# balazs-bamer/cdpr-simulation

Measured on AMD Instinct MI355X. Metric: CDPR sim-steps/sec (whole node), 65 536 parallel 8-cable robots, 1 ms dt, higher is better.
Workload: dtype f32

## Files before the change

cdpr-simulation_amd/csrc/cdpr_onestep_kernel.hpp:

```cpp
#pragma once
#include "cdpr_step_kernel.hpp"

namespace cdpr {

CDPR_DEV void row_to_lds(const float4* src, float4* dst_row) {
  __builtin_amdgcn_global_load_lds((const __attribute__((address_space(1))) void*)src, (__attribute__((address_space(3))) void*)dst_row, 16, 0, 0);
}


template <int NP, bool PR = false, bool FULL = false>
CDPR_DEV void pid_pairs(const StepArgs& a, int calls, bool is_vel, const v2f (&desired)[NP], const v2f (&actual)[NP], const v2f (&win)[NP][kWin],
                        v2f (&ierr)[NP], v2f (&f)[NP], v2f (&e_new)[NP], float& dbg_p, float& dbg_i, float& dbg_d, bool is_force = false) {
  const PidCoef c = pid_coef<PR>(a, is_vel);
  const bool run = (!PR || calls != 0) && !is_force;
  const bool full = FULL || calls >= c.nbuf;
  const float (&wt)[kWin + 2] = a.wrow;
  v2f error[NP], acc[NP];
#pragma unroll
  for (int k = 0; k < NP; ++k) {
    error[k] = desired[k] - actual[k];
    acc[k] = splat(wt[kWin]) * error[k];
  }
#pragma unroll
  for (int j = 0; j < kWin; ++j) {
// ... 328 lines not shown
      ik_pairs<N, false>(lds + again, s.px, s.py, s.pz, s.qx, s.qy, s.qz, s.qw, len2, jac, l02);
    }
    float w[6];
    jt_times<NP>(jac, tens, w);
    w[0] = a.fgx - w[0];
    w[1] = a.fgy - w[1];
    w[2] = a.fgz - w[2];
    w[3] = -w[3];
    w[4] = -w[4];
    w[5] = -w[5];
    integrate(a, s, w);
  }
  if (PERSIST && more) {
    constexpr int kDmaOps = kCtrl + kCmdRows;
    static_assert(kDmaOps < 64, "vmcnt is a 6-bit counter");
    if (run_pid)
      __builtin_amdgcn_s_waitcnt(vmcnt_imm(kDmaOps));
    else
      __builtin_amdgcn_s_waitcnt(vmcnt_imm(0));
    asm volatile("" : "+a"(n0), "+a"(n1), "+a"(n2), "+a"(n3), "+a"(n4));
  }
  if (live) {
    CDPR_STORE_STATE(a.state, st, 0, woff, make_float4(s.px, s.py, s.pz, s.qx));
    CDPR_STORE_STATE(a.state, st, 1, woff, make_float4(s.qy, s.qz, s.qw, s.vx));
    CDPR_STORE_STATE(a.state, st, 2, woff, make_float4(s.vy, s.vz, s.wx, s.wy));
    CDPR_STORE_STATE(a.state, st, 3, woff, make_float4(s.wz, fkx, fky, fkz));
    if (FK) CDPR_STORE_STATE(a.state, st, 4, woff, make_float4(fkqx, fkqy, fkqz, fkqw));
  }
  CDPR_STAMP(7);
  if (!(PERSIST && more)) break;
  blk = nblk;
  r = nr;
  rr = nrr;
  live = r < a.batch;
  off = rr * 16u, woff = r * 16u;
  p0 = make_float4(n0.x, n0.y, n0.z, n0.w), p1 = make_float4(n1.x, n1.y, n1.z, n1.w), p2 = make_float4(n2.x, n2.y, n2.z, n2.w);
  p3 = make_float4(n3.x, n3.y, n3.z, n3.w), p4 = make_float4(n4.x, n4.y, n4.z, n4.w);
  staged = run_pid;
  }
}

#ifndef CDPR_CTL_LOAD_DELAY
#define CDPR_CTL_LOAD_DELAY 8
#endif
#ifndef CDPR_SPLIT_PRIO
#define CDPR_SPLIT_PRIO 1
#endif
#ifndef CDPR_STEADY_SHARED_IK
#define CDPR_STEADY_SHARED_IK 1
#endif
#ifndef CDPR_STEADY_NEWTON_WRITTEN_OUT
#define CDPR_STEADY_NEWTON_WRITTEN_OUT 1
#endif
constexpr int kIkRows = 7;
#ifdef CDPR_STAMPS
#define CDPR_SPLIT_STAMP(i)                                                                                          \
  do {                                                                                                               \
    __builtin_amdgcn_sched_barrier(0);                                                                               \
    if (a.stamps && lane == 0) a.stamps[(size_t)blockIdx.x * 8 + (i)] = __builtin_amdgcn_s_memrealtime();           \
    __builtin_amdgcn_sched_barrier(0);                                                                               \
  } while (0)
#else
#define CDPR_SPLIT_STAMP(i) do { } while (0)
#endif
#if defined(CDPR_STAMPS) && defined(CDPR_STAMPS_ITER)
#define CDPR_CTL_STAMP(i) do { } while (0)
#else
#define CDPR_CTL_STAMP(i) CDPR_SPLIT_STAMP(i)
#endif

template <int N, int XS, int ES, bool RAISED = true, bool STEADY = false>
CDPR_DEV void split_estimator_wave(const StepArgs& a, float* geo, float gval, uint32_t lane, bool live, size_t st, uint32_t off, uint32_t woff,
                                   const float4& p0, const float4& p1, const float4& p3, const v2f* x_force, v2f* x_tension, float* x_est,
                                   v2f* x_ik = nullptr) {
  constexpr int NP = cable_pairs(N);
#if defined(CDPR_STAMPS) && defined(CDPR_STAMPS_CLOCK)
  const unsigned long long clk0 = __builtin_amdgcn_s_memtime();
#endif
#if CDPR_SPLIT_PRIO == 1 || CDPR_SPLIT_PRIO == 4
  if (RAISED) __builtin_amdgcn_s_setprio(3);
#elif CDPR_SPLIT_PRIO == 3 || CDPR_SPLIT_PRIO == 5
  if (RAISED) __builtin_amdgcn_s_setprio(2);
#endif
  const float4 p4 = load_slot(a.state, st, 4, off);
  if (lane < NP * kGeomFloatsPerPair) geo[lane] = gval;
  __builtin_amdgcn_fence(__ATOMIC_RELEASE, "wavefront");
  __builtin_amdgcn_wave_barrier();
  __builtin_amdgcn_fence(__ATOMIC_ACQUIRE, "wavefront");
  float fkx = p3.y, fky = p3.z, fkz = p3.w, fkqx = p4.x, fkqy = p4.y, fkqz = p4.z, fkqw = p4.w;
  v2f len[NP];
  {
    v2f jac[NP][6], l0[NP];
    ik_pairs<N, false>(geo, p0.x, p0.y, p0.z, p0.w, p1.x, p1.y, p1.z, len, jac, l0);
    if (STEADY && CDPR_STEADY_SHARED_IK) {
#pragma unroll
      for (int k = 0; k < NP; ++k) {
        x_ik[(kIkRows * k) * 64 + lane] = len[k];
#pragma unroll
        for (int c = 0; c < 6; ++c) x_ik[(kIkRows * k + 1 + c) * 64 + lane] = jac[k][c];
      }
      __builtin_amdgcn_fence(__ATOMIC_RELEASE, "workgroup");
      __builtin_amdgcn_s_waitcnt(0xC07F);
      __builtin_amdgcn_s_barrier();
    }
  }
  float fk_res = 0.f;
  int fk_it = 0;
  v2f jest[NP][6];
  {
    v2f elen[NP], unused[NP];
    if (STEADY && CDPR_STEADY_NEWTON_WRITTEN_OUT) {
#pragma unroll
      for (int it = 0; it < 4; ++it) {
        ik_pairs<N, false>(geo, fkx, fky, fkz, fkqx, fkqy, fkqz, fkqw, elen, jest, unused);
        v2f res[NP];
#pragma unroll
        for (int k = 0; k < NP; ++k) res[k] = len[k] - elen[k];
        float g[6];
        jt_times<NP>(jest, res, g);
        normal_solve<NP>(jest, a.fk_lambda, g);
        fkx += g[0];
        fky += g[1];
        fkz += g[2];
        quat_apply_rotvec(fkqx, fkqy, fkqz, fkqw, g[3], g[4], g[5]);
#ifdef CDPR_STAMPS_ITER
        if (it < 3) {
          asm volatile("" ::"v"(fkqw));
          __builtin_amdgcn_sched_barrier(0);
          if (a.stamps && lane == 0) a.stamps[(size_t)blockIdx.x * 8 + 4 + it] = __builtin_amdgcn_s_memrealtime();
          __builtin_amdgcn_sched_barrier(0);
        }
#endif
      }
      fk_it = 4;
    } else {
      bool active = true;
      for (int it = 0; it < a.fk_iters; ++it) {
        ik_pairs<N, false>(geo, fkx, fky, fkz, fkqx, fkqy, fkqz, fkqw, elen, jest, unused);
        v2f res[NP];
        v2f rm = splat(0.f);
#pragma unroll
        for (int k = 0; k < NP; ++k) {
          res[k] = len[k] - elen[k];
          rm = max2(rm, abs2(res[k]));
        }
        active = active && !(fmaxf(rm.x, rm.y) < a.fk_tol);
        float g[6];
        jt_times<NP>(jest, res, g);
        normal_solve<NP>(jest, a.fk_lambda, g);
        if (active) {
          fkx += g[0];
          fky += g[1];
          fkz += g[2];
          quat_apply_rotvec(fkqx, fkqy, fkqz, fkqw, g[3], g[4], g[5]);
          ++fk_it;
        }
#ifdef CDPR_STAMPS_ITER
        if (it < 3) {
          asm volatile("" ::"v"(fkqw));
          __builtin_amdgcn_sched_barrier(0);
          if (a.stamps && lane == 0) a.stamps[(size_t)blockIdx.x * 8 + 4 + it] = __builtin_amdgcn_s_memrealtime();
          __builtin_amdgcn_sched_barrier(0);
        }
#endif
      }
    }
    ik_pairs<N, false>(geo, fkx, fky, fkz, fkqx, fkqy, fkqz, fkqw, elen, jest, unused);
    v2f rm = splat(0.f);
#pragma unroll
    for (int k = 0; k < NP; ++k) rm = max2(rm, abs2(len[k] - elen[k]));
    fk_res = fmaxf(rm.x, rm.y);
  }
  if (live) store_slot_aux<CDPR_SPLIT_PLAT_AUX>(a.state, st, 4, woff, make_float4(fkqx, fkqy, fkqz, fkqw));
  CDPR_SPLIT_STAMP(1);
  v2f td_l[6][3];
  float td_invd[6];
  normal_matrix_pk<NP, false>(jest, 0.f, td_l);
  chol_factor_pk(td_l, td_invd);
  __builtin_amdgcn_s_waitcnt(0xC07F);
  __builtin_amdgcn_s_barrier();
  CDPR_SPLIT_STAMP(2);
  __builtin_amdgcn_fence(__ATOMIC_ACQUIRE, "workgroup");
  v2f f[NP], df[NP], t_out[NP];
#pragma unroll
  for (int k = 0; k < NP; ++k) {
    f[k] = x_force[k * XS + lane];
    df[k] = f[k] - splat(a.td_mid);
  }
  int td_flag = 0;
  {
    float g[6];
    jt_times<NP>(jest, df, g);
    chol_apply_pk(td_l, td_invd, g);
#pragma unroll
    for (int k = 0; k < NP; ++k) {
      v2f t = splat(a.td_mid);
#pragma unroll
      for (int c = 0; c < 6; ++c) t = fma2(g[c], jest[k][c], t);
      const v2f tc = max2(min2(t, splat(a.td_max)), splat(a.td_min));
      td_flag |= (tc.x != t.x) ? 1 : 0;
      if (2 * k + 1 < N) td_flag |= (tc.y != t.y) ? 1 : 0;
      t_out[k] = tc;
    }
  }
#pragma unroll
  for (int k = 0; k < NP; ++k) x_tension[k * XS + lane] = t_out[k];
  x_est[0 * ES + lane] = fkx;
  x_est[1 * ES + lane] = fky;
  x_est[2 * ES + lane] = fkz;
  x_est[3 * ES + lane] = fk_res;
  x_est[4 * ES + lane] = (float)fk_it;
  x_est[5 * ES + lane] = (float)td_flag;
  __builtin_amdgcn_fence(__ATOMIC_RELEASE, "workgroup");
  __builtin_amdgcn_s_waitcnt(0xC07F);
  CDPR_SPLIT_STAMP(3);
#if defined(CDPR_STAMPS) && defined(CDPR_STAMPS_CLOCK)
  if (a.stamps && lane == 0) a.stamps[(size_t)blockIdx.x * 8 + 7] = __builtin_amdgcn_s_memtime() - clk0;
#endif
  __builtin_amdgcn_s_barrier();
}

template <int N, bool PR, bool STEADY, bool VEL>
CDPR_DEV void split_controller_wave(const StepArgs& a, float* geo, float gval, uint32_t lane, uint32_t r, uint32_t rr, bool live, size_t st, uint32_t off,
                                    uint32_t woff, const float4& p0, const float4& p1, const float4& p2, const float4& p3, v2f* x_force, const v2f* x_tension,
                                    const float* x_est, const v2f* x_ik = nullptr) {
  static_assert(!(STEADY && PR), "the steady instantiation serves uniform handles");
  constexpr int NP = cable_pairs(N);
  constexpr int P = plat_slots(true);
  constexpr int G = joint_groups(N);
  constexpr int NH = (NP + 1) / 2;
#if CDPR_SPLIT_PRIO == 2 || CDPR_SPLIT_PRIO == 5
  __builtin_amdgcn_s_setprio(3);
#endif
#if CDPR_CTL_LOAD_DELAY > 0
  __builtin_amdgcn_s_sleep(CDPR_CTL_LOAD_DELAY);
#endif
  float4 wraw[NP][5], hraw[NH];
#pragma unroll
  for (int k = 0; k < NP; ++k) {
#pragma unroll
    for (int m = 0; m < 5; ++m) wraw[k][m] = load_slot(a.state, st, P + 5 * k + m, off);
  }
#pragma unroll
  for (int g = 0; g < NH; ++g) hraw[g] = load_slot(a.state, st, P + 5 * NP + g, off);
  v2f desired[NP];
#pragma unroll
  for (int k = 0; k < NP; ++k) desired[k] = splat(0.f);
  const float* cp = a.cmd + (size_t)rr * N;
  if (N % 4 == 0) {
#pragma unroll
    for (int g = 0; g < N / 4; ++g) {
      const float4 v = reinterpret_cast<const float4*>(cp)[g];
      desired[2 * g] = (v2f){v.x, v.y};
      desired[2 * g + 1] = (v2f){v.z, v.w};
    }
  } else {
#pragma unroll
    for (int i = 0; i < N; ++i) {
      if (i & 1)
        desired[i / 2].y = cp[i];
      else
        desired[i / 2].x = cp[i];
    }
  }
  if (lane < NP * kGeomFloatsPerPair) geo[lane] = gval;
  __builtin_amdgcn_fence(__ATOMIC_RELEASE, "wavefront");
  __builtin_amdgcn_wave_barrier();
  __builtin_amdgcn_fence(__ATOMIC_ACQUIRE, "wavefront");

  Platform s;
  unpack_platform(p0, p1, p2, p3.x, s);

  v2f len[NP], q[NP], qd[NP], jac[NP][6];
  {
    v2f l0[NP];
    if (STEADY && CDPR_STEADY_SHARED_IK) {
      __builtin_amdgcn_s_barrier();
      __builtin_amdgcn_fence(__ATOMIC_ACQUIRE, "workgroup");
#pragma unroll
      for (int k = 0; k < NP; ++k) {
        len[k] = x_ik[(kIkRows * k) * 64 + lane];
#pragma unroll
        for (int c = 0; c < 6; ++c) jac[k][c] = x_ik[(kIkRows * k + 1 + c) * 64 + lane];
        l0[k] = *reinterpret_cast<const v2f*>(geo + k * kGeomFloatsPerPair + 12);
      }
    } else {
      ik_pairs<N, true>(geo, s.px, s.py, s.pz, s.qx, s.qy, s.qz, s.qw, len, jac, l0);
    }
#pragma unroll
    for (int k = 0; k < NP; ++k) {
      q[k] = l0[k] - len[k];
      qd[k] = -fma2(s.wz, jac[k][5], fma2(s.wy, jac[k][4], fma2(s.wx, jac[k][3],
                    fma2(s.vz, jac[k][2], fma2(s.vy, jac[k][1], splat(s.vx) * jac[k][0])))));
    }
  }
  const bool publish = STEADY || (a.publish_mask & 1ull) != 0ull;
  if (publish && live) {
    store_slot(a.obs, st, 0, woff, make_float4(s.px, s.py, s.pz, s.qx));
    store_slot(a.obs, st, 1, woff, make_float4(s.qy, s.qz, s.qw, s.vx));
    store_slot(a.obs, st, 2, woff, make_float4(s.vy, s.vz, s.wx, s.wy));
#pragma unroll
    for (int g = 0; g < G; ++g) {
      const int k0 = 2 * g, k1 = (2 * g + 1 < NP) ? 2 * g + 1 : 2 * g;
      const bool has = (2 * g + 1 < NP);
      store_slot(a.obs, st, 4 + g, woff, make_float4(q[k0].x, q[k0].y, has ? q[k1].x : 0.f, has ? q[k1].y : 0.f));
      store_slot(a.obs, st, 4 + G + g, woff, make_float4(qd[k0].x, qd[k0].y, has ? qd[k1].x : 0.f, has ? qd[k1].y : 0.f));
    }
  }

  v2f f[NP], e_new[NP], ierr[NP];
#pragma unroll
  for (int k = 0; k < NP; ++k) {
    f[k] = splat(0.f);
    e_new[k] = splat(0.f);
    ierr[k] = (k & 1) ? (v2f){hraw[k / 2].z, hraw[k / 2].w} : (v2f){hraw[k / 2].x, hraw[k / 2].y};
  }
  float dbg_p = 0.f, dbg_i = 0.f, dbg_d = 0.f;
  bool dbg_wrote = false;
  const bool first_world = !STEADY && (a.flags & kFlagFirstWorldStep) != 0u;
  uint32_t meta = 0u;
  if (PR) meta = a.meta[rr];
  const int calls = PR ? (int)(meta >> kMetaCallShift) : a.pid_calls;
  if (PR && live && !first_world) a.meta[r] = (uint8_t)((meta & kMetaModeMask) | ((uint32_t)min(calls + 1, (int)kMetaCallMax) << kMetaCallShift));
  const bool force_mode = !STEADY && !PR && (a.flags & kFlagForceMode) != 0u;
  if (force_mode && !first_world) {
#pragma unroll
    for (int k = 0; k < NP; ++k) f[k] = desired[k];
  } else if (STEADY || (!first_world && (PR || calls != 0))) {
    v2f win[NP][kWin];
#pragma unroll
    for (int k = 0; k < NP; ++k) {
#pragma unroll
      for (int m = 0; m < 5; ++m) {
        win[k][2 * m] = (v2f){wraw[k][m].x, wraw[k][m].y};
        win[k][2 * m + 1] = (v2f){wraw[k][m].z, wraw[k][m].w};
      }
    }
    const bool actual_is_vel = STEADY ? VEL : PR ? ((meta & kMetaModeMask) == kMetaVelocity) : ((a.flags & kFlagActualIsVelocity) != 0u);
    v2f actual[NP];
#pragma unroll
    for (int k = 0; k < NP; ++k) actual[k] = actual_is_vel ? qd[k] : q[k];
    const int ring_slot = a.ring_slot;
    const bool is_force = PR && (meta & kMetaModeMask) == kMetaForce;
#if CDPR_SPLIT_PRIO == 3 || CDPR_SPLIT_PRIO == 4
    __builtin_amdgcn_s_setprio(3);
#endif
    pid_pairs<NP, PR, STEADY>(a, calls, actual_is_vel, desired, actual, win, ierr, f, e_new, dbg_p, dbg_i, dbg_d, is_force);
    dbg_wrote = (!PR || calls != 0) && !is_force;
    if (live) {
#pragma unroll
      for (int m = 0; m < 5; ++m) {
        if (m == (ring_slot >> 1)) {
          if (!STEADY) {
#pragma unroll
            for (int k = 0; k < NP; ++k) CDPR_STORE_STATE(a.state, st, P + 5 * k + m, woff, ring_row(win[k], m, e_new[k], ring_slot));
          } else if (ring_slot & 1) {
#pragma unroll
            for (int k = 0; k < NP; ++k) CDPR_STORE_STATE(a.state, st, P + 5 * k + m, woff, make_float4(win[k][2 * m].x, win[k][2 * m].y, e_new[k].x, e_new[k].y));
          } else {
#pragma unroll
            for (int k = 0; k < NP; ++k) CDPR_STORE_STATE(a.state, st, P + 5 * k + m, woff, make_float4(e_new[k].x, e_new[k].y, win[k][2 * m + 1].x, win[k][2 * m + 1].y));
          }
        }
      }
#pragma unroll
      for (int g = 0; g < NH; ++g) {
        const int k1 = (2 * g + 1 < NP) ? 2 * g + 1 : 2 * g;
        CDPR_STORE_STATE(a.state, st, P + 5 * NP + g, woff, make_float4(ierr[2 * g].x, ierr[2 * g].y, ierr[k1].x, ierr[k1].y));
      }
    }
  }
#pragma unroll
  for (int k = 0; k < NP; ++k) x_force[k * 64 + lane] = f[k];
  __builtin_amdgcn_fence(__ATOMIC_RELEASE, "workgroup");
  __builtin_amdgcn_s_waitcnt(0xC07F);
  CDPR_CTL_STAMP(4);
#if CDPR_SPLIT_PRIO >= 3
  __builtin_amdgcn_s_setprio(0);
#endif
  __builtin_amdgcn_s_barrier();
  __builtin_amdgcn_s_barrier();
  CDPR_CTL_STAMP(5);
  __builtin_amdgcn_fence(__ATOMIC_ACQUIRE, "workgroup");
  v2f applied[NP];
#pragma unroll
  for (int k = 0; k < NP; ++k) applied[k] = x_tension[k * 64 + lane];
  const float fkx = x_est[0 * 64 + lane], fky = x_est[1 * 64 + lane], fkz = x_est[2 * 64 + lane], fk_res = x_est[3 * 64 + lane],
              fk_it = x_est[4 * 64 + lane], td_flag = x_est[5 * 64 + lane];
  setforce_limits<NP>(a, qd, applied);
  if (!STEADY && a.dbg && live) write_pid_topic(a.dbg + (size_t)r * 9, dbg_wrote, dbg_wrote, dbg_p, dbg_i, dbg_d, desired[0].x, applied[0].x);
  if (publish && live) {
    store_slot(a.obs, st, 3, woff, make_float4(s.wz, fk_res, fk_it, (!STEADY && a.travel_on) ? pack_flags((int)td_flag, travel_mask<N>(a, q)) : td_flag));
#pragma unroll
    for (int g = 0; g < G; ++g) {
      const int k0 = 2 * g, k1 = (2 * g + 1 < NP) ? 2 * g + 1 : 2 * g;
      const bool has = (2 * g + 1 < NP);
      store_slot(a.obs, st, 4 + 2 * G + g, woff,
                 make_float4(applied[k0].x, applied[k0].y, has ? applied[k1].x : 0.f, has ? applied[k1].y : 0.f));
    }
  }
  {
    v2f tens[NP];
#pragma unroll
    for (int k = 0; k < NP; ++k) {
      tens[k] = fma2(-a.damping, qd[k], applied[k]);
      if (a.unilateral) tens[k] = max2(tens[k], splat(0.f));
    }
    float w[6];
    jt_times<NP>(jac, tens, w);
    w[0] = a.fgx - w[0];
    w[1] = a.fgy - w[1];
    w[2] = a.fgz - w[2];
    w[3] = -w[3];
    w[4] = -w[4];
    w[5] = -w[5];
    integrate(a, s, w);
  }
  if (live) {
    store_slot_aux<CDPR_SPLIT_PLAT_AUX>(a.state, st, 0, woff, make_float4(s.px, s.py, s.pz, s.qx));
    store_slot_aux<CDPR_SPLIT_PLAT_AUX>(a.state, st, 1, woff, make_float4(s.qy, s.qz, s.qw, s.vx));
    store_slot_aux<CDPR_SPLIT_PLAT_AUX>(a.state, st, 2, woff, make_float4(s.vy, s.vz, s.wx, s.wy));
    store_slot_aux<CDPR_SPLIT_PLAT_AUX>(a.state, st, 3, woff, make_float4(s.wz, fkx, fky, fkz));
  }
  CDPR_CTL_STAMP(6);
}

template <int N, bool PR, bool STEADY, bool VEL>
CDPR_DEV void split_kernel_body(const StepArgs& a) {
  constexpr int NP = cable_pairs(N);
  __shared__ __attribute__((aligned(16))) float lds[2][NP * kGeomFloatsPerPair];
  __shared__ v2f x_force[NP][64];
  __shared__ v2f x_tension[NP][64];
  __shared__ float x_est[6][64];
  v2f* x_ik = nullptr;
  if constexpr (STEADY && CDPR_STEADY_SHARED_IK) {
    __shared__ v2f ik_rows_at_state[kIkRows * NP][64];
    x_ik = &ik_rows_at_state[0][0];
  }

  const uint32_t swap = __builtin_popcount(blockIdx.x & a.split_swap) & 1u;
  const uint32_t wave = (threadIdx.x >> 6) ^ swap, lane = threadIdx.x & 63u;
  const uint32_t r = blockIdx.x * 64u + lane;
  const uint32_t rr = (r < a.batch) ? r : (a.batch - 1u);
  const bool live = r < a.batch;
  const size_t st = a.stride;
  const uint32_t off = rr * 16u, woff = r * 16u;
  float* const geo = lds[wave];

  if (wave == 0) CDPR_SPLIT_STAMP(0);
#ifdef CDPR_STAMPS
  if (a.stamps && lane == 0)
    reinterpret_cast<uint32_t*>(&a.stamps[(size_t)blockIdx.x * 8 + 7])[threadIdx.x >> 6] =
        (__builtin_amdgcn_s_getreg((16 - 1) << 11 | 4) & 0xffffu) | ((__builtin_amdgcn_s_getreg((4 - 1) << 11 | 20) & 0xfu) << 16);
#endif
  const float gval = (lane < NP * kGeomFloatsPerPair) ? a.geom[lane] : 0.f;
  const float4 p0 = load_slot(a.state, st, 0, off), p1 = load_slot(a.state, st, 1, off), p2 = load_slot(a.state, st, 2, off),
               p3 = load_slot(a.state, st, 3, off);
  if (wave == 0) {
    split_estimator_wave<N, 64, 64, true, STEADY>(a, geo, gval, lane, live, st, off, woff, p0, p1, p3, &x_force[0][0], &x_tension[0][0], &x_est[0][0], x_ik);
    return;
  }
  split_controller_wave<N, PR, STEADY, VEL>(a, geo, gval, lane, r, rr, live, st, off, woff, p0, p1, p2, p3, &x_force[0][0], &x_tension[0][0], &x_est[0][0], x_ik);
}
template <int N, bool PR = false>
__global__ __launch_bounds__(128, 2) void cdpr_split_kernel(const StepArgs a) { split_kernel_body<N, PR, false, false>(a); }
template <int N, bool VEL>
__global__ __launch_bounds__(128, 2) void cdpr_split_steady_kernel(const StepArgs a) { split_kernel_body<N, false, true, VEL>(a); }

}
```

cdpr-simulation_amd/csrc/cdpr_step_kernel.hpp:

```cpp
#pragma once
#include <hip/hip_runtime.h>
#include <stdint.h>

namespace cdpr {

constexpr int kMaxCables = 8;
constexpr int kWin = 10;
constexpr int kGeomFloatsPerPair = 16;

typedef float v2f __attribute__((ext_vector_type(2)));

enum StepFlags : uint32_t {
  kFlagFirstWorldStep = 1u << 0,
  kFlagRolloutResetPid = 1u << 1,
  kFlagActualIsVelocity = 1u << 2,
  kFlagPublishAll = 1u << 4,
  kFlagForceMode = 1u << 3,
};

struct PidSet {
  float kf, kp, ki, kd, inv_ki, imax, imin, cmax, cmin;
  int clamp_cmd;
};

// ... 77 lines not shown

#ifdef CDPR_STAMPS
#define CDPR_STAMP(i)                                                                           \
  do {                                                                                          \
    __builtin_amdgcn_sched_barrier(0);                                                          \
    if (a.stamps && threadIdx.x == 0) a.stamps[(size_t)blockIdx.x * 8 + (i)] = __builtin_amdgcn_s_memrealtime(); \
    __builtin_amdgcn_sched_barrier(0);                                                          \
  } while (0)
#else
#define CDPR_STAMP(i) do { } while (0)
#endif

#ifdef CDPR_LEAF_NODEBUG
#define CDPR_LEAF __device__ __forceinline__ __attribute__((nodebug))
#else
#define CDPR_LEAF CDPR_DEV
#endif
CDPR_LEAF v2f splat(float s) { return (v2f){s, s}; }
CDPR_LEAF v2f fma2(v2f a, v2f b, v2f c) { return __builtin_elementwise_fma(a, b, c); }
CDPR_LEAF v2f fma2(float a, v2f b, v2f c) { return __builtin_elementwise_fma(splat(a), b, c); }
CDPR_LEAF float hsum(v2f v) {
  float r;
  asm("v_add_f32_e32 %0, %1, %2" : "=v"(r) : "v"(v.x), "v"(v.y));
  return r;
}
CDPR_DEV v2f rsq2(v2f v) { return (v2f){__frsqrt_rn(v.x), __frsqrt_rn(v.y)}; }
CDPR_LEAF v2f min2(v2f a, v2f b) { return (v2f){fminf(a.x, b.x), fminf(a.y, b.y)}; }
CDPR_LEAF v2f max2(v2f a, v2f b) { return (v2f){fmaxf(a.x, b.x), fmaxf(a.y, b.y)}; }
CDPR_LEAF v2f abs2(v2f a) { return (v2f){fabsf(a.x), fabsf(a.y)}; }
CDPR_LEAF float comp4(const float4& v, int k) { return k == 0 ? v.x : (k == 1 ? v.y : (k == 2 ? v.z : v.w)); }

struct Rot {
  float r00, r01, r02, r10, r11, r12, r20, r21, r22;
};

CDPR_DEV Rot quat_to_rot(float x, float y, float z, float w) {
  const float x2 = x + x, y2 = y + y, z2 = z + z;
  const float xx = x * x2, yy = y * y2, zz = z * z2;
  const float xy = x * y2, xz = x * z2, yz = y * z2;
  const float wx = w * x2, wy = w * y2, wz = w * z2;
  Rot r;
  r.r00 = 1.f - (yy + zz);
  r.r01 = xy - wz;
  r.r02 = xz + wy;
  r.r10 = xy + wz;
  r.r11 = 1.f - (xx + zz);
  r.r12 = yz - wx;
  r.r20 = xz - wy;
  r.r21 = yz + wx;
  r.r22 = 1.f - (xx + yy);
  return r;
}

CDPR_DEV void quat_apply_rotvec(float& qx, float& qy, float& qz, float& qw, float tx, float ty, float tz) {
  const float a2 = fmaf(tz, tz, fmaf(ty, ty, tx * tx));
  const float inv_a = __frsqrt_rn(fmaxf(a2, 1e-30f));
  float s, c;
  __sincosf(0.5f * (a2 * inv_a), &s, &c);
  const bool tiny = a2 < 1e-8f;
  const float k = tiny ? fmaf(a2, -1.f / 48.f, 0.5f) : s * inv_a;
  const float cw = tiny ? fmaf(a2, -0.125f, 1.f) : c;
  const float dx = k * tx, dy = k * ty, dz = k * tz;
  const float nw = fmaf(-dz, qz, fmaf(-dy, qy, fmaf(-dx, qx, cw * qw)));
  const float nx = fmaf(-dz, qy, fmaf(dy, qz, fmaf(qw, dx, cw * qx)));
  const float ny = fmaf(-dx, qz, fmaf(dz, qx, fmaf(qw, dy, cw * qy)));
  const float nz = fmaf(-dy, qx, fmaf(dx, qy, fmaf(qw, dz, cw * qz)));
  const float inv = __frsqrt_rn(fmaf(nw, nw, fmaf(nz, nz, fmaf(ny, ny, nx * nx))));
  qx = nx * inv;
  qy = ny * inv;
  qz = nz * inv;
  qw = nw * inv;
}

template <int NP, bool ODD, bool WANT_L0>
CDPR_DEV void ik_rows(const float* lds, float px, float py, float pz, float qx, float qy, float qz, float qw,
                      v2f (&len)[NP], v2f (&jac)[NP][6], v2f (&l0)[NP]) {
  const Rot r = quat_to_rot(qx, qy, qz, qw);
#pragma unroll
  for (int k = 0; k < NP; ++k) {
    const float4 g0 = *reinterpret_cast<const float4*>(lds + k * kGeomFloatsPerPair);
    const float4 g1 = *reinterpret_cast<const float4*>(lds + k * kGeomFloatsPerPair + 4);
    const float4 g2 = *reinterpret_cast<const float4*>(lds + k * kGeomFloatsPerPair + 8);
    const v2f ax = {g0.x, g0.y}, ay = {g0.z, g0.w}, az = {g1.x, g1.y};
    const v2f bx = {g1.z, g1.w}, by = {g2.x, g2.y}, bz = {g2.z, g2.w};
    const v2f rbx = fma2(r.r02, bz, fma2(r.r01, by, splat(r.r00) * bx));
    const v2f rby = fma2(r.r12, bz, fma2(r.r11, by, splat(r.r10) * bx));
    const v2f rbz = fma2(r.r22, bz, fma2(r.r21, by, splat(r.r20) * bx));
    const v2f lx = (rbx - ax) + splat(px), ly = (rby - ay) + splat(py), lz = (rbz - az) + splat(pz);
    const v2f l2 = fma2(lz, lz, fma2(ly, ly, lx * lx));
    const v2f inv = rsq2(l2);
    len[k] = l2 * inv;
    const v2f ux = lx * inv, uy = ly * inv, uz = lz * inv;
    jac[k][0] = ux;
    jac[k][1] = uy;
    jac[k][2] = uz;
    jac[k][3] = fma2(rby, uz, -(rbz * uy));
    jac[k][4] = fma2(rbz, ux, -(rbx * uz));
    jac[k][5] = fma2(rbx, uy, -(rby * ux));
    if (WANT_L0 || (ODD && k == NP - 1)) {
      const float4 g3 = *reinterpret_cast<const float4*>(lds + k * kGeomFloatsPerPair + 12);
      l0[k] = (v2f){g3.x, g3.y};
      if (ODD && k == NP - 1) {
        const v2f mask = {g3.z, g3.w};
        len[k] *= mask;
#pragma unroll
        for (int c = 0; c < 6; ++c) jac[k][c] *= mask;
      }
    }
  }
}

template <int N, bool WANT_L0>
CDPR_DEV void ik_pairs(const float* lds, float px, float py, float pz, float qx, float qy, float qz, float qw,
                       v2f (&len)[cable_pairs(N)], v2f (&jac)[cable_pairs(N)][6], v2f (&l0)[cable_pairs(N)]) {
  ik_rows<cable_pairs(N), (N & 1) != 0, WANT_L0>(lds, px, py, pz, qx, qy, qz, qw, len, jac, l0);
}

template <int NP>
CDPR_DEV void jt_partial(const v2f (&jac)[NP][6], const v2f (&v)[NP], v2f (&acc)[6]) {
#pragma unroll
  for (int c = 0; c < 6; ++c) acc[c] = jac[0][c] * v[0];
#pragma unroll
  for (int k = 1; k < NP; ++k) {
#pragma unroll
    for (int c = 0; c < 6; ++c) acc[c] = fma2(jac[k][c], v[k], acc[c]);
  }
}

template <int NP>
CDPR_DEV void jt_times(const v2f (&jac)[NP][6], const v2f (&v)[NP], float (&g)[6]) {
  v2f acc[6];
  jt_partial<NP>(jac, v, acc);
#pragma unroll
  for (int c = 0; c < 6; ++c) g[c] = hsum(acc[c]);
}

template <int NP>
CDPR_DEV void gram_partial(const v2f (&jac)[NP][6], v2f (&acc)[21]) {
#pragma unroll
  for (int a = 0, e = 0; a < 6; ++a) {
#pragma unroll
    for (int b = 0; b <= a; ++b, ++e) acc[e] = jac[0][a] * jac[0][b];
  }
#pragma unroll
  for (int k = 1; k < NP; ++k) {
#pragma unroll
    for (int a = 0, e = 0; a < 6; ++a) {
#pragma unroll
      for (int b = 0; b <= a; ++b, ++e) acc[e] = fma2(jac[k][a], jac[k][b], acc[e]);
    }
  }
}

CDPR_DEV void chol_solve(float (&m)[6][6], float (&g)[6]) {
  float invd[6];
#pragma unroll
  for (int j = 0; j < 6; ++j) {
    float d = m[j][j];
#pragma unroll
    for (int k = 0; k < j; ++k) d = fmaf(-m[j][k], m[j][k], d);
    invd[j] = __frsqrt_rn(d);
#pragma unroll
    for (int i = j + 1; i < 6; ++i) {
      float s = m[i][j];
#pragma unroll
      for (int k = 0; k < j; ++k) s = fmaf(-m[i][k], m[j][k], s);
      m[i][j] = s * invd[j];
    }
  }
#pragma unroll
// ... 75 lines not shown
  mp[5][2].x = 0.f;
}

template <int NP, bool LAMBDA = true>
CDPR_DEV void normal_solve(const v2f (&jac)[NP][6], float lambda, float (&g)[6]) {
#if CDPR_CHOL_PACKED
  v2f mp[6][3];
  normal_matrix_pk<NP, LAMBDA>(jac, lambda, mp);
  chol_solve_pk(mp, g);
#else
  v2f acc[21];
  gram_partial<NP>(jac, acc);
  float m[6][6];
#pragma unroll
  for (int a = 0, e = 0; a < 6; ++a) {
#pragma unroll
    for (int b = 0; b <= a; ++b, ++e) m[a][b] = (LAMBDA && a == b) ? hsum(acc[e]) + lambda : hsum(acc[e]);
  }
  chol_solve(m, g);
#endif
}

struct PidCoef {
  float kf, kp, ki, kd, inv_ki, imax, imin, cmax, cmin;
  int nbuf;
  bool clamp;
};
template <bool PR>
CDPR_DEV PidCoef pid_coef(const StepArgs& a, bool is_vel) {
  PidCoef c;
  const bool alt = PR && !is_vel;
  c.kf = alt ? a.alt.kf : a.kf;
  c.kp = alt ? a.alt.kp : a.kp;
  c.ki = alt ? a.alt.ki : a.ki;
  c.kd = alt ? a.alt.kd : a.kd;
  c.inv_ki = alt ? a.alt.inv_ki : a.inv_ki;
  c.imax = alt ? a.alt.imax : a.imax;
  c.imin = alt ? a.alt.imin : a.imin;
  c.cmax = alt ? a.alt.cmax : a.cmax;
  c.cmin = alt ? a.alt.cmin : a.cmin;
  c.nbuf = a.nbuf;
  c.clamp = (alt ? a.alt.clamp_cmd : a.clamp_cmd) != 0;
  return c;
}
constexpr uint32_t kMetaModeMask = 3u, kMetaCallShift = 2u, kMetaCallMax = 63u;
constexpr uint32_t kMetaForce = 0u, kMetaPosition = 1u, kMetaVelocity = 2u;

struct Platform {
  float px, py, pz, qx, qy, qz, qw;
  float vx, vy, vz, wx, wy, wz;
};

CDPR_DEV void integrate_pose(const StepArgs& a, Platform& s);
CDPR_DEV void integrate_velocity(const StepArgs& a, Platform& s, const float (&w)[6]) {
  const Rot r = quat_to_rot(s.qx, s.qy, s.qz, s.qw);
  s.vx = fmaf(a.dt_inv_mass, w[0], s.vx);
  s.vy = fmaf(a.dt_inv_mass, w[1], s.vy);
  s.vz = fmaf(a.dt_inv_mass, w[2], s.vz);
  float tbx = fmaf(r.r20, w[5], fmaf(r.r10, w[4], r.r00 * w[3]));
  float tby = fmaf(r.r21, w[5], fmaf(r.r11, w[4], r.r01 * w[3]));
  float tbz = fmaf(r.r22, w[5], fmaf(r.r12, w[4], r.r02 * w[3]));
  const float obx = fmaf(r.r20, s.wz, fmaf(r.r10, s.wy, r.r00 * s.wx));
  const float oby = fmaf(r.r21, s.wz, fmaf(r.r11, s.wy, r.r01 * s.wx));
  const float obz = fmaf(r.r22, s.wz, fmaf(r.r12, s.wy, r.r02 * s.wx));
  const float iox = fmaf(a.ib[4], obz, fmaf(a.ib[3], oby, a.ib[0] * obx));
  const float ioy = fmaf(a.ib[5], obz, fmaf(a.ib[1], oby, a.ib[3] * obx));
  const float ioz = fmaf(a.ib[2], obz, fmaf(a.ib[5], oby, a.ib[4] * obx));
  tbx -= fmaf(oby, ioz, -(obz * ioy));
  tby -= fmaf(obz, iox, -(obx * ioz));
  tbz -= fmaf(obx, ioy, -(oby * iox));
  const float abx = fmaf(a.ibinv[4], tbz, fmaf(a.ibinv[3], tby, a.ibinv[0] * tbx));
  const float aby = fmaf(a.ibinv[5], tbz, fmaf(a.ibinv[1], tby, a.ibinv[3] * tbx));
  const float abz = fmaf(a.ibinv[2], tbz, fmaf(a.ibinv[5], tby, a.ibinv[4] * tbx));
  s.wx = fmaf(a.dt, fmaf(r.r02, abz, fmaf(r.r01, aby, r.r00 * abx)), s.wx);
  s.wy = fmaf(a.dt, fmaf(r.r12, abz, fmaf(r.r11, aby, r.r10 * abx)), s.wy);
  s.wz = fmaf(a.dt, fmaf(r.r22, abz, fmaf(r.r21, aby, r.r20 * abx)), s.wz);
}

CDPR_DEV void integrate_pose(const StepArgs& a, Platform& s) {
  s.px = fmaf(a.dt, s.vx, s.px);
  s.py = fmaf(a.dt, s.vy, s.py);
  s.pz = fmaf(a.dt, s.vz, s.pz);
  const float h = a.half_dt;
  const float nx = fmaf(h, fmaf(-s.wz, s.qy, fmaf(s.wy, s.qz, s.qw * s.wx)), s.qx);
  const float ny = fmaf(h, fmaf(-s.wx, s.qz, fmaf(s.wz, s.qx, s.qw * s.wy)), s.qy);
  const float nz = fmaf(h, fmaf(-s.wy, s.qx, fmaf(s.wx, s.qy, s.qw * s.wz)), s.qz);
  const float nw = fmaf(-h, fmaf(s.wz, s.qz, fmaf(s.wy, s.qy, s.wx * s.qx)), s.qw);
  const float inv = __frsqrt_rn(fmaf(nw, nw, fmaf(nz, nz, fmaf(ny, ny, nx * nx))));
  s.qx = nx * inv;
  s.qy = ny * inv;
  s.qz = nz * inv;
  s.qw = nw * inv;
}

CDPR_DEV void integrate(const StepArgs& a, Platform& s, const float (&w)[6]) {
  integrate_velocity(a, s, w);
  integrate_pose(a, s);
}

template <int N>
CDPR_DEV uint32_t travel_mask(const StepArgs& a, const v2f (&q)[cable_pairs(N)]) {
  uint32_t m = 0u;
  if (a.travel_on) {
#pragma unroll
    for (int k = 0; k < cable_pairs(N); ++k) {
      m |= (q[k].x < a.travel_lo || q[k].x > a.travel_hi) ? (1u << (2 * k)) : 0u;
      if (2 * k + 1 < N) m |= (q[k].y < a.travel_lo || q[k].y > a.travel_hi) ? (1u << (2 * k + 1)) : 0u;
    }
  }
  return m;
}
CDPR_DEV float pack_flags(int td_flag, uint32_t limit_mask) { return (float)((uint32_t)td_flag | (limit_mask << 1)); }

template <int N>
CDPR_DEV void apply_travel_stop(const StepArgs& a, Platform& s, const v2f (&q)[cable_pairs(N)], const v2f (&jac)[cable_pairs(N)][6]) {
  const Rot r = quat_to_rot(s.qx, s.qy, s.qz, s.qw);
  float vx = s.vx, vy = s.vy, vz = s.vz, wx = s.wx, wy = s.wy, wz = s.wz;
  for (int sweep = 0; sweep < a.travel_stop; ++sweep)
#pragma unroll
  for (int i = 0; i < N; ++i) {
    const int k = i / 2;
    float j[6];
#pragma unroll
    for (int c = 0; c < 6; ++c) j[c] = (i & 1) ? jac[k][c].y : jac[k][c].x;
    const float qi = (i & 1) ? q[k].y : q[k].x;
    const float qdn = -fmaf(j[5], wz, fmaf(j[4], wy, fmaf(j[3], wx, fmaf(j[2], vz, fmaf(j[1], vy, j[0] * vx)))));
    const bool hit = (qi >= a.travel_hi && qdn > 0.f) || (qi <= a.travel_lo && qdn < 0.f);
    const float tbx = fmaf(r.r20, j[5], fmaf(r.r10, j[4], r.r00 * j[3]));
    const float tby = fmaf(r.r21, j[5], fmaf(r.r11, j[4], r.r01 * j[3]));
    const float tbz = fmaf(r.r22, j[5], fmaf(r.r12, j[4], r.r02 * j[3]));
    const float abx = fmaf(a.ibinv[4], tbz, fmaf(a.ibinv[3], tby, a.ibinv[0] * tbx));
    const float aby = fmaf(a.ibinv[5], tbz, fmaf(a.ibinv[1], tby, a.ibinv[3] * tbx));
    const float abz = fmaf(a.ibinv[2], tbz, fmaf(a.ibinv[5], tby, a.ibinv[4] * tbx));
    const float awx = fmaf(r.r02, abz, fmaf(r.r01, aby, r.r00 * abx));
    const float awy = fmaf(r.r12, abz, fmaf(r.r11, aby, r.r10 * abx));
    const float awz = fmaf(r.r22, abz, fmaf(r.r21, aby, r.r20 * abx));
    const float d = fmaf(j[5], awz, fmaf(j[4], awy, fmaf(j[3], awx, fmaf(j[2], j[2], fmaf(j[1], j[1], j[0] * j[0])) * a.inv_mass)));
    const float lam = hit ? qdn / d : 0.f;
    const float lm = lam * a.inv_mass;
    vx = fmaf(lm, j[0], vx);
    vy = fmaf(lm, j[1], vy);
    vz = fmaf(lm, j[2], vz);
    wx = fmaf(lam, awx, wx);
    wy = fmaf(lam, awy, wy);
    wz = fmaf(lam, awz, wz);
  }
  s.vx = vx, s.vy = vy, s.vz = vz, s.wx = wx, s.wy = wy, s.wz = wz;
}

// ... 666 lines not shown
```

Baseline: 6.817 billion.

## Pack quaternion math into v_pk ops and share rotation matrix via LDS

Adds packed-f32 versions of quaternion-to-rotation, rotation-vector update and the cable IK rows, built on v_pk_add/v_pk_fma with op_sel and neg modifiers. These are used in the estimator's Newton loop and in the true-state IK. In the steady kernel, the estimator wave writes the true-state rotation matrix to LDS so the controller wave can reuse it in integration instead of recomputing it. It also skips writing a constant iteration count and pins the Cholesky factor with an empty asm statement. The cost is more LDS traffic and hand-written inline asm that the compiler cannot schedule around.

Result: faster. 7.007 billion, median of 6 (+2.8%).

```diff
diff --git a/cdpr-simulation_amd/csrc/cdpr_onestep_kernel.hpp b/cdpr-simulation_amd/csrc/cdpr_onestep_kernel.hpp
--- a/cdpr-simulation_amd/csrc/cdpr_onestep_kernel.hpp
+++ b/cdpr-simulation_amd/csrc/cdpr_onestep_kernel.hpp
@@ -404,7 +404,57 @@
 #ifndef CDPR_STEADY_NEWTON_WRITTEN_OUT
 #define CDPR_STEADY_NEWTON_WRITTEN_OUT 1
 #endif
+#ifndef CDPR_EST_PIN_FACTOR
+#define CDPR_EST_PIN_FACTOR 1
+#endif
+#ifndef CDPR_STEADY_SHARED_ROT
+#define CDPR_STEADY_SHARED_ROT 1
+#endif
 constexpr int kIkRows = 7;
+constexpr bool kSteadySharedRot = CDPR_STEADY_SHARED_IK && CDPR_STEADY_SHARED_ROT;
+
+struct EstQuat {
+  v2f a, b;
+};
+CDPR_DEV EstQuat est_quat(const float4& v) { return EstQuat{(v2f){v.x, v.y}, (v2f){v.z, v.w}}; }
+CDPR_DEV float4 est_quat_row(const EstQuat& q) { return make_float4(q.a.x, q.a.y, q.b.x, q.b.y); }
+template <int N>
+CDPR_DEV void est_ik(const float* geo, float x, float y, float z, const EstQuat& q, v2f (&len)[cable_pairs(N)], v2f (&jac)[cable_pairs(N)][6],
+                     v2f (&l0)[cable_pairs(N)]) {
+#if CDPR_QUAT_PK
+  ik_pairs_pk<N, false>(geo, x, y, z, quat_to_rot_pk(q.a, q.b), len, jac, l0);
+#else
+  ik_pairs<N, false>(geo, x, y, z, q.a.x, q.a.y, q.b.x, q.b.y, len, jac, l0);
+#endif
+}
+CDPR_DEV void est_rotate(EstQuat& q, float tx, float ty, float tz) {
+#if CDPR_QUAT_PK
+  quat_apply_rotvec_pk(q.a, q.b, tx, ty, tz);
+#else
+  float x = q.a.x, y = q.a.y, z = q.b.x, w = q.b.y;
+  quat_apply_rotvec(x, y, z, w, tx, ty, tz);
+  q = EstQuat{(v2f){x, y}, (v2f){z, w}};
+#endif
+}
+CDPR_DEV Rot true_state_rot(float qx, float qy, float qz, float qw) {
+#if CDPR_QUAT_PK
+  return unpack_rot(quat_to_rot_pk((v2f){qx, qy}, (v2f){qz, qw}));
+#else
+  return quat_to_rot(qx, qy, qz, qw);
+#endif
+}
+template <int N, bool WANT_L0>
+CDPR_DEV Rot true_state_ik(const float* geo, float px, float py, float pz, float qx, float qy, float qz, float qw, v2f (&len)[cable_pairs(N)],
+                           v2f (&jac)[cable_pairs(N)][6], v2f (&l0)[cable_pairs(N)]) {
+#if CDPR_QUAT_PK
+  const RotPk r = quat_to_rot_pk((v2f){qx, qy}, (v2f){qz, qw});
+  ik_pairs_pk<N, WANT_L0>(geo, px, py, pz, r, len, jac, l0);
+  return unpack_rot(r);
+#else
+  ik_pairs<N, WANT_L0>(geo, px, py, pz, qx, qy, qz, qw, len, jac, l0);
+  return quat_to_rot(qx, qy, qz, qw);
+#endif
+}
 #ifdef CDPR_STAMPS
 #define CDPR_SPLIT_STAMP(i)                                                                                          \
   do {                                                                                                               \
@@ -424,7 +474,7 @@
 template <int N, int XS, int ES, bool RAISED = true, bool STEADY = false>
 CDPR_DEV void split_estimator_wave(const StepArgs& a, float* geo, float gval, uint32_t lane, bool live, size_t st, uint32_t off, uint32_t woff,
                                    const float4& p0, const float4& p1, const float4& p3, const v2f* x_force, v2f* x_tension, float* x_est,
-                                   v2f* x_ik = nullptr) {
+                                   v2f* x_ik = nullptr, float* x_rot = nullptr) {
   constexpr int NP = cable_pairs(N);
 #if defined(CDPR_STAMPS) && defined(CDPR_STAMPS_CLOCK)
   const unsigned long long clk0 = __builtin_amdgcn_s_memtime();
@@ -439,12 +489,22 @@
   __builtin_amdgcn_fence(__ATOMIC_RELEASE, "wavefront");
   __builtin_amdgcn_wave_barrier();
   __builtin_amdgcn_fence(__ATOMIC_ACQUIRE, "wavefront");
-  float fkx = p3.y, fky = p3.z, fkz = p3.w, fkqx = p4.x, fkqy = p4.y, fkqz = p4.z, fkqw = p4.w;
+  float fkx = p3.y, fky = p3.z, fkz = p3.w;
+  EstQuat fkq = est_quat(p4);
   v2f len[NP];
   {
     v2f jac[NP][6], l0[NP];
-    ik_pairs<N, false>(geo, p0.x, p0.y, p0.z, p0.w, p1.x, p1.y, p1.z, len, jac, l0);
+    float tqx = p0.w, tqy = p1.x, tqz = p1.y, tqw = p1.z;
+#if CDPR_QUAT_PK
+    asm volatile("" : "+v"(tqx), "+v"(tqy), "+v"(tqz), "+v"(tqw));
+#endif
+    const Rot r = true_state_ik<N, false>(geo, p0.x, p0.y, p0.z, tqx, tqy, tqz, tqw, len, jac, l0);
     if (STEADY && CDPR_STEADY_SHARED_IK) {
+      if (kSteadySharedRot) {
+        x_rot[0 * 64 + lane] = r.r00, x_rot[1 * 64 + lane] = r.r01, x_rot[2 * 64 + lane] = r.r02;
+        x_rot[3 * 64 + lane] = r.r10, x_rot[4 * 64 + lane] = r.r11, x_rot[5 * 64 + lane] = r.r12;
+        x_rot[6 * 64 + lane] = r.r20, x_rot[7 * 64 + lane] = r.r21, x_rot[8 * 64 + lane] = r.r22;
+      }
 #pragma unroll
       for (int k = 0; k < NP; ++k) {
         x_ik[(kIkRows * k) * 64 + lane] = len[k];
@@ -464,7 +524,7 @@
     if (STEADY && CDPR_STEADY_NEWTON_WRITTEN_OUT) {
 #pragma unroll
       for (int it = 0; it < 4; ++it) {
-        ik_pairs<N, false>(geo, fkx, fky, fkz, fkqx, fkqy, fkqz, fkqw, elen, jest, unused);
+        est_ik<N>(geo, fkx, fky, fkz, fkq, elen, jest, unused);
         v2f res[NP];
 #pragma unroll
         for (int k = 0; k < NP; ++k) res[k] = len[k] - elen[k];
@@ -474,10 +534,10 @@
         fkx += g[0];
         fky += g[1];
         fkz += g[2];
-        quat_apply_rotvec(fkqx, fkqy, fkqz, fkqw, g[3], g[4], g[5]);
+        est_rotate(fkq, g[3], g[4], g[5]);
 #ifdef CDPR_STAMPS_ITER
         if (it < 3) {
-          asm volatile("" ::"v"(fkqw));
+          asm volatile("" ::"v"(est_quat_row(fkq).w));
           __builtin_amdgcn_sched_barrier(0);
           if (a.stamps && lane == 0) a.stamps[(size_t)blockIdx.x * 8 + 4 + it] = __builtin_amdgcn_s_memrealtime();
           __builtin_amdgcn_sched_barrier(0);
@@ -488,7 +548,7 @@
     } else {
       bool active = true;
       for (int it = 0; it < a.fk_iters; ++it) {
-        ik_pairs<N, false>(geo, fkx, fky, fkz, fkqx, fkqy, fkqz, fkqw, elen, jest, unused);
+        est_ik<N>(geo, fkx, fky, fkz, fkq, elen, jest, unused);
         v2f res[NP];
         v2f rm = splat(0.f);
 #pragma unroll
@@ -504,12 +564,12 @@
           fkx += g[0];
           fky += g[1];
           fkz += g[2];
-          quat_apply_rotvec(fkqx, fkqy, fkqz, fkqw, g[3], g[4], g[5]);
+          est_rotate(fkq, g[3], g[4], g[5]);
           ++fk_it;
         }
 #ifdef CDPR_STAMPS_ITER
         if (it < 3) {
-          asm volatile("" ::"v"(fkqw));
+          asm volatile("" ::"v"(est_quat_row(fkq).w));
           __builtin_amdgcn_sched_barrier(0);
           if (a.stamps && lane == 0) a.stamps[(size_t)blockIdx.x * 8 + 4 + it] = __builtin_amdgcn_s_memrealtime();
           __builtin_amdgcn_sched_barrier(0);
@@ -517,18 +577,21 @@
 #endif
       }
     }
-    ik_pairs<N, false>(geo, fkx, fky, fkz, fkqx, fkqy, fkqz, fkqw, elen, jest, unused);
+    est_ik<N>(geo, fkx, fky, fkz, fkq, elen, jest, unused);
     v2f rm = splat(0.f);
 #pragma unroll
     for (int k = 0; k < NP; ++k) rm = max2(rm, abs2(len[k] - elen[k]));
     fk_res = fmaxf(rm.x, rm.y);
   }
-  if (live) store_slot_aux<CDPR_SPLIT_PLAT_AUX>(a.state, st, 4, woff, make_float4(fkqx, fkqy, fkqz, fkqw));
+  if (live) store_slot_aux<CDPR_SPLIT_PLAT_AUX>(a.state, st, 4, woff, est_quat_row(fkq));
   CDPR_SPLIT_STAMP(1);
   v2f td_l[6][3];
   float td_invd[6];
   normal_matrix_pk<NP, false>(jest, 0.f, td_l);
   chol_factor_pk(td_l, td_invd);
+#if CDPR_EST_PIN_FACTOR
+  asm volatile("" ::"v"(td_invd[5]), "v"(fk_res));
+#endif
   __builtin_amdgcn_s_waitcnt(0xC07F);
   __builtin_amdgcn_s_barrier();
   CDPR_SPLIT_STAMP(2);
@@ -561,7 +624,7 @@
   x_est[1 * ES + lane] = fky;
   x_est[2 * ES + lane] = fkz;
   x_est[3 * ES + lane] = fk_res;
-  x_est[4 * ES + lane] = (float)fk_it;
+  if (!STEADY) x_est[4 * ES + lane] = (float)fk_it;
   x_est[5 * ES + lane] = (float)td_flag;
   __builtin_amdgcn_fence(__ATOMIC_RELEASE, "workgroup");
   __builtin_amdgcn_s_waitcnt(0xC07F);
@@ -575,7 +638,7 @@
 template <int N, bool PR, bool STEADY, bool VEL>
 CDPR_DEV void split_controller_wave(const StepArgs& a, float* geo, float gval, uint32_t lane, uint32_t r, uint32_t rr, bool live, size_t st, uint32_t off,
                                     uint32_t woff, const float4& p0, const float4& p1, const float4& p2, const float4& p3, v2f* x_force, const v2f* x_tension,
-                                    const float* x_est, const v2f* x_ik = nullptr) {
+                                    const float* x_est, const v2f* x_ik = nullptr, const float* x_rot = nullptr) {
   static_assert(!(STEADY && PR), "the steady instantiation serves uniform handles");
   constexpr int NP = cable_pairs(N);
   constexpr int P = plat_slots(true);
@@ -624,9 +687,11 @@
   unpack_platform(p0, p1, p2, p3.x, s);
 
   v2f len[NP], q[NP], qd[NP], jac[NP][6];
+  constexpr bool kOwnIk = !(STEADY && CDPR_STEADY_SHARED_IK);
+  Rot rot;
   {
     v2f l0[NP];
-    if (STEADY && CDPR_STEADY_SHARED_IK) {
+    if (!kOwnIk) {
       __builtin_amdgcn_s_barrier();
       __builtin_amdgcn_fence(__ATOMIC_ACQUIRE, "workgroup");
 #pragma unroll
@@ -637,7 +702,7 @@
         l0[k] = *reinterpret_cast<const v2f*>(geo + k * kGeomFloatsPerPair + 12);
       }
     } else {
-      ik_pairs<N, true>(geo, s.px, s.py, s.pz, s.qx, s.qy, s.qz, s.qw, len, jac, l0);
+      rot = true_state_ik<N, true>(geo, s.px, s.py, s.pz, s.qx, s.qy, s.qz, s.qw, len, jac, l0);
     }
 #pragma unroll
     for (int k = 0; k < NP; ++k) {
@@ -738,7 +803,15 @@
 #pragma unroll
   for (int k = 0; k < NP; ++k) applied[k] = x_tension[k * 64 + lane];
   const float fkx = x_est[0 * 64 + lane], fky = x_est[1 * 64 + lane], fkz = x_est[2 * 64 + lane], fk_res = x_est[3 * 64 + lane],
-              fk_it = x_est[4 * 64 + lane], td_flag = x_est[5 * 64 + lane];
+              fk_it = STEADY ? 4.f : x_est[4 * 64 + lane], td_flag = x_est[5 * 64 + lane];
+  if (!kOwnIk) {
+    if (kSteadySharedRot) {
+      rot = Rot{x_rot[0 * 64 + lane], x_rot[1 * 64 + lane], x_rot[2 * 64 + lane], x_rot[3 * 64 + lane], x_rot[4 * 64 + lane],
+                x_rot[5 * 64 + lane], x_rot[6 * 64 + lane], x_rot[7 * 64 + lane], x_rot[8 * 64 + lane]};
+    } else {
+      rot = true_state_rot(s.qx, s.qy, s.qz, s.qw);
+    }
+  }
   setforce_limits<NP>(a, qd, applied);
   if (!STEADY && a.dbg && live) write_pid_topic(a.dbg + (size_t)r * 9, dbg_wrote, dbg_wrote, dbg_p, dbg_i, dbg_d, desired[0].x, applied[0].x);
   if (publish && live) {
@@ -766,7 +839,7 @@
     w[3] = -w[3];
     w[4] = -w[4];
     w[5] = -w[5];
-    integrate(a, s, w);
+    integrate(a, s, w, rot);
   }
   if (live) {
     store_slot_aux<CDPR_SPLIT_PLAT_AUX>(a.state, st, 0, woff, make_float4(s.px, s.py, s.pz, s.qx));
@@ -785,9 +858,14 @@
   __shared__ v2f x_tension[NP][64];
   __shared__ float x_est[6][64];
   v2f* x_ik = nullptr;
+  float* x_rot = nullptr;
   if constexpr (STEADY && CDPR_STEADY_SHARED_IK) {
     __shared__ v2f ik_rows_at_state[kIkRows * NP][64];
     x_ik = &ik_rows_at_state[0][0];
+    if constexpr (kSteadySharedRot) {
+      __shared__ float rot_at_state[9][64];
+      x_rot = &rot_at_state[0][0];
+    }
   }
 
   const uint32_t swap = __builtin_popcount(blockIdx.x & a.split_swap) & 1u;
@@ -809,10 +887,10 @@
   const float4 p0 = load_slot(a.state, st, 0, off), p1 = load_slot(a.state, st, 1, off), p2 = load_slot(a.state, st, 2, off),
                p3 = load_slot(a.state, st, 3, off);
   if (wave == 0) {
-    split_estimator_wave<N, 64, 64, true, STEADY>(a, geo, gval, lane, live, st, off, woff, p0, p1, p3, &x_force[0][0], &x_tension[0][0], &x_est[0][0], x_ik);
+    split_estimator_wave<N, 64, 64, true, STEADY>(a, geo, gval, lane, live, st, off, woff, p0, p1, p3, &x_force[0][0], &x_tension[0][0], &x_est[0][0], x_ik, x_rot);
     return;
   }
-  split_controller_wave<N, PR, STEADY, VEL>(a, geo, gval, lane, r, rr, live, st, off, woff, p0, p1, p2, p3, &x_force[0][0], &x_tension[0][0], &x_est[0][0], x_ik);
+  split_controller_wave<N, PR, STEADY, VEL>(a, geo, gval, lane, r, rr, live, st, off, woff, p0, p1, p2, p3, &x_force[0][0], &x_tension[0][0], &x_est[0][0], x_ik, x_rot);
 }
 template <int N, bool PR = false>
 __global__ __launch_bounds__(128, 2) void cdpr_split_kernel(const StepArgs a) { split_kernel_body<N, PR, false, false>(a); }
diff --git a/cdpr-simulation_amd/csrc/cdpr_step_kernel.hpp b/cdpr-simulation_amd/csrc/cdpr_step_kernel.hpp
--- a/cdpr-simulation_amd/csrc/cdpr_step_kernel.hpp
+++ b/cdpr-simulation_amd/csrc/cdpr_step_kernel.hpp
@@ -153,6 +153,70 @@
   return r;
 }
 
+#ifndef CDPR_QUAT_PK
+#define CDPR_QUAT_PK 1
+#endif
+
+CDPR_LEAF v2f lo2(v2f v) { return __builtin_shufflevector(v, v, 0, 0); }
+CDPR_LEAF v2f hi2(v2f v) { return __builtin_shufflevector(v, v, 1, 1); }
+CDPR_LEAF v2f swap2(v2f v) { return __builtin_shufflevector(v, v, 1, 0); }
+CDPR_LEAF v2f pk_add_swap_neg_hi(v2f a, v2f b) {
+  v2f r;
+  asm("v_pk_add_f32 %0, %1, %2 op_sel:[0,1] op_sel_hi:[1,0] neg_hi:[0,1]" : "=v"(r) : "v"(a), "v"(b));
+  return r;
+}
+CDPR_LEAF v2f pk_add_swap_neg_lo(v2f a, v2f b) {
+  v2f r;
+  asm("v_pk_add_f32 %0, %1, %2 op_sel:[0,1] op_sel_hi:[1,0] neg_lo:[0,1]" : "=v"(r) : "v"(a), "v"(b));
+  return r;
+}
+CDPR_LEAF v2f pk_lo_minus_plus_hi(v2f a, v2f b) {
+  v2f r;
+  asm("v_pk_add_f32 %0, %1, %2 op_sel:[0,1] op_sel_hi:[0,1] neg_lo:[0,1]" : "=v"(r) : "v"(a), "v"(b));
+  return r;
+}
+CDPR_LEAF v2f pk_fma_hi_neg_hi(v2f a, v2f b, v2f c) {
+  v2f r;
+  asm("v_pk_fma_f32 %0, %1, %2, %3 op_sel:[0,1,0] op_sel_hi:[1,1,1] neg_hi:[1,0,0]" : "=v"(r) : "v"(a), "v"(b), "v"(c));
+  return r;
+}
+
+CDPR_LEAF float fma_half(float a, float b, float c) {
+  float r;
+  asm("v_fma_f32 %0, %1, %2, %3" : "=v"(r) : "v"(a), "v"(b), "v"(c));
+  return r;
+}
+CDPR_LEAF float fnma_half(float a, float b, float c) {
+  float r;
+  asm("v_fma_f32 %0, -%1, %2, %3" : "=v"(r) : "v"(a), "v"(b), "v"(c));
+  return r;
+}
+
+struct RotPk {
+  v2f d;
+  v2f o;
+  v2f c;
+  v2f l;
+  float r22;
+};
+CDPR_DEV Rot unpack_rot(const RotPk& p) { return Rot{p.d.x, p.o.x, p.c.x, p.o.y, p.d.y, p.c.y, p.l.x, p.l.y, p.r22}; }
+
+CDPR_DEV RotPk quat_to_rot_pk(v2f A, v2f B) {
+  const v2f T = A + A, U = B + B;
+  const v2f P1 = A * T;
+  const v2f P2 = A * lo2(U);
+  const v2f P3 = hi2(B) * T;
+  const v2f P4 = B * lo2(U);
+  const v2f XY = A * swap2(T);
+  RotPk r;
+  r.c = pk_add_swap_neg_hi(P2, P3);
+  r.l = pk_add_swap_neg_lo(P2, P3);
+  r.o = pk_lo_minus_plus_hi(XY, P4);
+  r.d = splat(1.f) - (swap2(P1) + lo2(P4));
+  r.r22 = 1.f - (P1.x + P1.y);
+  return r;
+}
+
 CDPR_DEV void quat_apply_rotvec(float& qx, float& qy, float& qz, float& qw, float tx, float ty, float tz) {
   const float a2 = fmaf(tz, tz, fmaf(ty, ty, tx * tx));
   const float inv_a = __frsqrt_rn(fmaxf(a2, 1e-30f));
@@ -171,6 +235,33 @@
   qy = ny * inv;
   qz = nz * inv;
   qw = nw * inv;
+}
+
+CDPR_DEV void quat_apply_rotvec_pk(v2f& A, v2f& B, float tx, float ty, float tz) {
+  const float a2 = fmaf(tz, tz, fmaf(ty, ty, tx * tx));
+  const float inv_a = __frsqrt_rn(fmaxf(a2, 1e-30f));
+  float s, c;
+  __sincosf(0.5f * (a2 * inv_a), &s, &c);
+  const bool tiny = a2 < 1e-8f;
+  const float k = tiny ? fmaf(a2, -1.f / 48.f, 0.5f) : s * inv_a;
+  const float cw = tiny ? fmaf(a2, -0.125f, 1.f) : c;
+  const v2f D = splat(k) * (v2f){tx, ty};
+  const float dz = k * tz;
+  v2f NA = splat(cw) * A;
+  NA = fma2(hi2(B), D, NA);
+  NA.x = fma_half(D.y, B.x, NA.x);
+  NA.y = fma_half(dz, A.x, NA.y);
+  NA.x = fnma_half(dz, A.y, NA.x);
+  NA.y = fnma_half(D.x, B.x, NA.y);
+  v2f NB = splat(cw) * B;
+  NB.x = fma_half(B.y, dz, NB.x);
+  NB.y = fnma_half(D.x, A.x, NB.y);
+  NB = pk_fma_hi_neg_hi(D, A, NB);
+  NB.x = fnma_half(D.y, A.x, NB.x);
+  NB.y = fnma_half(dz, B.x, NB.y);
+  const float inv = __frsqrt_rn(fmaf(NB.y, NB.y, fmaf(NB.x, NB.x, fmaf(NA.y, NA.y, NA.x * NA.x))));
+  A = NA * splat(inv);
+  B = NB * splat(inv);
 }
 
 template <int NP, bool ODD, bool WANT_L0>
@@ -217,6 +308,47 @@
   ik_rows<cable_pairs(N), (N & 1) != 0, WANT_L0>(lds, px, py, pz, qx, qy, qz, qw, len, jac, l0);
 }
 
+template <int NP, bool ODD, bool WANT_L0>
+CDPR_DEV void ik_rows_pk(const float* lds, float px, float py, float pz, const RotPk& r, v2f (&len)[NP], v2f (&jac)[NP][6], v2f (&l0)[NP]) {
+#pragma unroll
+  for (int k = 0; k < NP; ++k) {
+    const float4 g0 = *reinterpret_cast<const float4*>(lds + k * kGeomFloatsPerPair);
+    const float4 g1 = *reinterpret_cast<const float4*>(lds + k * kGeomFloatsPerPair + 4);
+    const float4 g2 = *reinterpret_cast<const float4*>(lds + k * kGeomFloatsPerPair + 8);
+    const v2f ax = {g0.x, g0.y}, ay = {g0.z, g0.w}, az = {g1.x, g1.y};
+    const v2f bx = {g1.z, g1.w}, by = {g2.x, g2.y}, bz = {g2.z, g2.w};
+    const v2f rbx = fma2(lo2(r.c), bz, fma2(lo2(r.o), by, lo2(r.d) * bx));
+    const v2f rby = fma2(hi2(r.c), bz, fma2(hi2(r.d), by, hi2(r.o) * bx));
+    const v2f rbz = fma2(r.r22, bz, fma2(hi2(r.l), by, lo2(r.l) * bx));
+    const v2f lx = (rbx - ax) + splat(px), ly = (rby - ay) + splat(py), lz = (rbz - az) + splat(pz);
+    const v2f l2 = fma2(lz, lz, fma2(ly, ly, lx * lx));
+    const v2f inv = rsq2(l2);
+    len[k] = l2 * inv;
+    const v2f ux = lx * inv, uy = ly * inv, uz = lz * inv;
+    jac[k][0] = ux;
+    jac[k][1] = uy;
+    jac[k][2] = uz;
+    jac[k][3] = fma2(rby, uz, -(rbz * uy));
+    jac[k][4] = fma2(rbz, ux, -(rbx * uz));
+    jac[k][5] = fma2(rbx, uy, -(rby * ux));
+    if (WANT_L0 || (ODD && k == NP - 1)) {
+      const float4 g3 = *reinterpret_cast<const float4*>(lds + k * kGeomFloatsPerPair + 12);
+      l0[k] = (v2f){g3.x, g3.y};
+      if (ODD && k == NP - 1) {
+        const v2f mask = {g3.z, g3.w};
+        len[k] *= mask;
+#pragma unroll
+        for (int c = 0; c < 6; ++c) jac[k][c] *= mask;
+      }
+    }
+  }
+}
+template <int N, bool WANT_L0>
+CDPR_DEV void ik_pairs_pk(const float* lds, float px, float py, float pz, const RotPk& r, v2f (&len)[cable_pairs(N)],
+                          v2f (&jac)[cable_pairs(N)][6], v2f (&l0)[cable_pairs(N)]) {
+  ik_rows_pk<cable_pairs(N), (N & 1) != 0, WANT_L0>(lds, px, py, pz, r, len, jac, l0);
+}
+
 template <int NP>
 CDPR_DEV void jt_partial(const v2f (&jac)[NP][6], const v2f (&v)[NP], v2f (&acc)[6]) {
 #pragma unroll
@@ -398,8 +530,7 @@
 };
 
 CDPR_DEV void integrate_pose(const StepArgs& a, Platform& s);
-CDPR_DEV void integrate_velocity(const StepArgs& a, Platform& s, const float (&w)[6]) {
-  const Rot r = quat_to_rot(s.qx, s.qy, s.qz, s.qw);
+CDPR_DEV void integrate_velocity(const StepArgs& a, Platform& s, const float (&w)[6], const Rot& r) {
   s.vx = fmaf(a.dt_inv_mass, w[0], s.vx);
   s.vy = fmaf(a.dt_inv_mass, w[1], s.vy);
   s.vz = fmaf(a.dt_inv_mass, w[2], s.vz);
@@ -422,6 +553,9 @@
   s.wy = fmaf(a.dt, fmaf(r.r12, abz, fmaf(r.r11, aby, r.r10 * abx)), s.wy);
   s.wz = fmaf(a.dt, fmaf(r.r22, abz, fmaf(r.r21, aby, r.r20 * abx)), s.wz);
 }
+CDPR_DEV void integrate_velocity(const StepArgs& a, Platform& s, const float (&w)[6]) {
+  integrate_velocity(a, s, w, quat_to_rot(s.qx, s.qy, s.qz, s.qw));
+}
 
 CDPR_DEV void integrate_pose(const StepArgs& a, Platform& s) {
   s.px = fmaf(a.dt, s.vx, s.px);
@@ -441,6 +575,10 @@
 
 CDPR_DEV void integrate(const StepArgs& a, Platform& s, const float (&w)[6]) {
   integrate_velocity(a, s, w);
+  integrate_pose(a, s);
+}
+CDPR_DEV void integrate(const StepArgs& a, Platform& s, const float (&w)[6], const Rot& r) {
+  integrate_velocity(a, s, w, r);
   integrate_pose(a, s);
 }
 
```
